# imuncle/TSCM_Calib

Measured on AMD Instinct MI355X. Metric: LM iterations/sec at 4 cams x 10k views (joint intrinsics+extrinsics, fp64), higher is better.
Workload: dtype f64

## Files before the change

### include/tscm/tscm.h

```cpp
#ifndef TSCM_H
#define TSCM_H

#include <stddef.h>

#ifdef __cplusplus
extern "C" {
#endif

#define TSCM_ABI_VERSION 6

enum {
    TSCM_OK = 0,
    TSCM_E_INVALID = -1,
    TSCM_E_NO_DEVICE = -2,
    TSCM_E_HIP = -3,
    TSCM_E_RCCL = -4,
    TSCM_E_UNSUPPORTED = -5,
    TSCM_E_NOMEM = -6,
    TSCM_E_PEER = -7
};

enum { TSCM_CONVERGENCE = 0, TSCM_NO_CONVERGENCE = 1, TSCM_FAILURE = 2 };

#define TSCM_MAX_ITERATIONS 255

typedef struct tscm_problem {
    int n_cameras;
    int n_boards;
    int n_points;
    int n_views;
    const double *board_xy;
    const int *view_camera;
    const int *view_board;
    const int *view_offset;
    const int *view_count;
    const double *obs_u;
    const double *obs_v;
    double *cam_rt;
    double *intr;
    double *board_rt;
    const unsigned char *cam_pose_constant;
    int mono;
    const unsigned char *board_pose_constant;
} tscm_problem;

typedef struct tscm_options {
    size_t struct_size;
    int max_num_iterations;
    double function_tolerance;
    double gradient_tolerance;
    double parameter_tolerance;
    double initial_trust_region_radius;
    double max_trust_region_radius;
    double min_trust_region_radius;
    double min_relative_decrease;
    double min_lm_diagonal;
    double max_lm_diagonal;
    int max_num_consecutive_invalid_steps;
    int jacobi_scaling;
    int check_every;
    int jacobian_fp32;
    int exec_flags;
} tscm_options;

enum {
    TSCM_EXEC_SEPARATE_T_REDUCE = 1,
    TSCM_EXEC_KEEP_SINGLE_RANK_COMM = 2,
    TSCM_EXEC_GRAM_16X16 = 4,
    TSCM_EXEC_SEPARATE_BACKSUB = 8,
    TSCM_EXEC_SEPARATE_CONTROL = 16,
    TSCM_EXEC_DENSE_REDUCED_ORDER = 32,
    TSCM_EXEC_GRAPH_REDUCED_ORDER = 64,
    TSCM_EXEC_SEPARATE_STATS = 128,
    TSCM_EXEC_ALL = 255
};

typedef struct tscm_iteration {
    int iteration;
    int step_is_valid;
    int step_is_successful;
    double cost;
    double cost_change;
    double gradient_max_norm;
    double gradient_norm;
    double step_norm;
    double relative_decrease;
    double trust_region_radius;
} tscm_iteration;

typedef struct tscm_summary {
    int termination_type;
    int num_iterations;
    int num_successful_steps;
    int num_unsuccessful_steps;
    double initial_cost;
    double final_cost;
    int n_residual_blocks;
    int lm_iterations;
    tscm_iteration iterations[TSCM_MAX_ITERATIONS + 1];
    char message[128];
    double seconds_solve;
    double seconds_total;
    double rmse;
} tscm_summary;

typedef struct tscm_solver tscm_solver;
typedef struct tscm_comm tscm_comm;

int tscm_abi_version(void);
const char *tscm_last_error(void);
int tscm_device_count(void);
int tscm_device_synchronize(int device);
int tscm_device_peak_fp64(int device, double *mfma_tflops, double *valu_tflops);
int tscm_device_peak_fp64_ex(int device, double peaks[3]);
int tscm_device_peak_fp32_mfma(int device, double *tflops);

void tscm_default_options(tscm_options *opt, int mono);

int tscm_solver_create(const tscm_problem *problem, int device, tscm_solver **out);
int tscm_solver_set_comm(tscm_solver *s, tscm_comm *comm);
int tscm_solver_debug_withhold_handoff(tscm_solver *s, int on);
int tscm_solver_reruns(const tscm_solver *s);
int tscm_solver_solve(tscm_solver *s, const tscm_options *opt, tscm_summary *summary);
int tscm_solver_upload_params(tscm_solver *s, const double *cam_rt, const double *intr, const double *board_rt);
int tscm_solver_solve_resident(tscm_solver *s, const tscm_options *opt, tscm_summary *summary, int reset);
int tscm_solver_download_params(tscm_solver *s, double *cam_rt, double *intr, double *board_rt);
void tscm_solver_destroy(tscm_solver *s);
// ... 253 lines not shown
```

### tscm_calib_amd/csrc/tscm_exec_plan.h

```cpp
#ifndef TSCM_EXEC_PLAN_H
#define TSCM_EXEC_PLAN_H

#include "tscm_layout.h"

#include <algorithm>
#include <string>

#ifdef __HIPCC__
#define TSCM_PLAN_FN __host__ __device__ inline
#else
#define TSCM_PLAN_FN inline
#endif

namespace tscm {

constexpr int kCamSl = 16;
constexpr int kTSlices = 16;
constexpr int kTEntries = 64;
constexpr int kFusedEntries = 256 / kTSlices;
constexpr int kVPrepThreads = 128;
constexpr int kDense4Cams = 4;

constexpr int kCtlOneGpu = 1;
constexpr int kCtlComm = 2;
constexpr int kCtlInit = 4;
constexpr int kCtlRide = 8;
constexpr int kCtlWithhold = 16;

enum CommKind { kCommNone, kCommOneRank, kCommShared };
inline bool uses_comm(int kind, int exec_flags) { return kind == kCommShared || (kind == kCommOneRank && (exec_flags & TSCM_EXEC_KEEP_SINGLE_RANK_COMM)); }

enum class Gram { G4, F32, G16, G16Pitch58 };
enum class EvalTail {
    ReduceControl,
    StatsThenHead,
    Ride,
    Exchange,
};
enum class Solver { Empty, Dense4, Nd, Big };

struct ExecDevice {
    int schur_resident[4] = {}, schur_resident_ride[4] = {};
    int dense4_resident = 0;
    int nd_resident[2] = {}, nd_tpt[2] = { 1, 1 };
};

struct ExecPlan {
    bool comm = false;
    Gram gram = Gram::G4;
    bool robust = false;
    EvalTail tail = EvalTail::ReduceControl;
    bool ctl_in_schur = false;
    bool stats_ride = false;
    bool t_in_solve = false;
    Solver solver = Solver::Empty;
    int nd = 0, tpt = 1;
    int n_prod = 0, n_bs = 0;
    int bs_threads = 0;
    bool f32() const { return gram == Gram::F32; }
};

inline int reduction_blocks(const Layout &L, int C) { return C * kCamSl + (L.B + 255) / 256; }

inline Gram plan_gram(int exec_flags, int jacobian_fp32, int rp)
{
    if (jacobian_fp32) return Gram::F32;
    if (!(exec_flags & TSCM_EXEC_GRAM_16X16)) return Gram::G4;
    return rp == 58 ? Gram::G16Pitch58 : Gram::G16;
}

constexpr int kG4MaxKS = 14;
struct G4Plan { int passes, per, ks; };
TSCM_PLAN_FN G4Plan g4_plan(int n_points)
{
    G4Plan g;
    g.passes = (n_points + 4 * kG4MaxKS - 1) / (4 * kG4MaxKS);
    if (g.passes < 1) g.passes = 1;
    g.ks = ((n_points + g.passes - 1) / g.passes + 3) / 4;
    if (g.ks < 1) g.ks = 1;
    g.per = 4 * g.ks;
    return g;
}

inline ExecPlan plan_exec(const Layout &L, int C, int n_act, int comm_kind, int exec_flags, int jacobian_fp32, int loss_kind, int rp,
                          const ExecDevice &dev)
{
    ExecPlan p;
    p.comm = uses_comm(comm_kind, exec_flags);
    p.gram = plan_gram(exec_flags, jacobian_fp32, rp);
    p.robust = loss_kind != TSCM_LOSS_NONE;
    const int n_variants = (L.nv_chunks[1] ? 1 : 0) + (L.nv_chunks[2] ? 1 : 0) + (L.nv_chunks[3] ? 1 : 0);
    const bool small = C <= kMaxCamLds;
    p.ctl_in_schur = (p.comm || small) && L.slow_boards.empty() && L.pc_begin.empty() && n_variants == 1 &&
                     !(exec_flags & TSCM_EXEC_SEPARATE_CONTROL);
    const int nv = L.nv_chunks[1] ? 1 : L.nv_chunks[2] ? 2 : 3;
    p.stats_ride = p.ctl_in_schur && !p.comm && small && !(exec_flags & TSCM_EXEC_SEPARATE_STATS) &&
                   std::max(reduction_blocks(L, C), L.nv_chunks[nv]) + 1 <= dev.schur_resident_ride[nv];
    p.tail = p.comm || !small ? EvalTail::Exchange : !p.ctl_in_schur ? EvalTail::ReduceControl : p.stats_ride ? EvalTail::Ride : EvalTail::StatsThenHead;
    p.t_in_solve = !(exec_flags & TSCM_EXEC_SEPARATE_T_REDUCE) && small && !p.comm && L.n_bids > 0 && L.n_bids <= kSmallBids && n_act > 0;
    p.n_prod = p.t_in_solve ? L.n_bids * (256 / kFusedEntries) : 0;
    p.nd = (exec_flags & TSCM_EXEC_DENSE_REDUCED_ORDER) ? 1 : 0;
    const bool graph_order = (exec_flags & TSCM_EXEC_GRAPH_REDUCED_ORDER) || p.nd;
    p.solver = n_act == 0 ? Solver::Empty : C <= kDense4Cams && !graph_order ? Solver::Dense4 : small ? Solver::Nd : Solver::Big;
    if (p.solver != Solver::Nd) p.nd = 0;
    p.tpt = p.solver == Solver::Nd ? dev.nd_tpt[p.nd] : 1;
    if (p.solver == Solver::Dense4 || p.solver == Solver::Nd) {
        const int resident = p.solver == Solver::Dense4 ? dev.dense4_resident : dev.nd_resident[p.nd];
        if (!(exec_flags & TSCM_EXEC_SEPARATE_BACKSUB) && L.bs_threads == 256 && L.n_bs_blocks <= resident - 1 - p.n_prod) p.n_bs = L.n_bs_blocks;
    }
    p.bs_threads = !p.n_bs && L.n_bs_blocks ? L.bs_threads : 0;
    return p;
}

inline int check_exec_options(const tscm_options &o, int loss_kind, std::string &err)
{
    if (o.max_num_iterations < 0 || o.max_num_iterations > TSCM_MAX_ITERATIONS) return layout_fail(err, TSCM_E_INVALID, "max_num_iterations must be in [0, 255]");
    if (o.exec_flags & ~TSCM_EXEC_ALL) return layout_fail(err, TSCM_E_INVALID, "unknown bits in tscm_options.exec_flags (an options struct of an older ABI?)");
    if (loss_kind != TSCM_LOSS_NONE && (o.exec_flags & TSCM_EXEC_GRAM_16X16)) return layout_fail(err, TSCM_E_UNSUPPORTED, "TSCM_EXEC_GRAM_16X16 has no robust-loss kernel");
    return 0;
}

}

#endif
```

### tscm_calib_amd/csrc/tscm_kernels.h

```cpp
#pragma once

#include "tscm_math.h"
#include "tscm_fastmath.h"
#include "tscm_nd_plan.h"
#include "tscm_layout.h"
#include "tscm_exec_plan.h"
#include "tscm_columns.h"
#include "tscm_ctrl.h"

namespace tscm {
#include "tscm_dev.h"
#include "tscm_probe.h"
#include "tscm_prep.h"
#include "tscm_geometry.h"
#include "tscm_eval_gram16.h"
#include "tscm_eval_f32.h"
#include "tscm_eval_gram4.h"
#include "tscm_reduce.h"
#include "tscm_schur.h"
#include "tscm_backsub.h"
#include "tscm_solve_nd.h"
#include "tscm_solve_dense4.h"
#include "tscm_solve_big.h"
#include "tscm_begin_end.h"
#include "tscm_ops.h"

}
```

### tscm_calib_amd/csrc/tscm_schur.h

```cpp
#pragma once

__device__ __forceinline__ bool chol6(const double M[21], double L[21])
{
    bool ok = true;
#pragma unroll
    for (int j = 0; j < 6; ++j) {
        double d = M[j * (j + 1) / 2 + j];
#pragma unroll
        for (int k = 0; k < j; ++k) d -= L[j * (j + 1) / 2 + k] * L[j * (j + 1) / 2 + k];
        if (!(d > 0.0)) { ok = false; d = 1.0; }
        const double inv = fast_rsqrt(d);
        L[j * (j + 1) / 2 + j] = inv;
#pragma unroll
        for (int i = j + 1; i < 6; ++i) {
            double s = M[i * (i + 1) / 2 + j];
#pragma unroll
            for (int k = 0; k < j; ++k) s -= L[i * (i + 1) / 2 + k] * L[j * (j + 1) / 2 + k];
            L[i * (i + 1) / 2 + j] = s * inv;
        }
    }
    return ok;
}

__device__ __forceinline__ bool factor_core(double (&M)[21], const double (&g)[6], const double (&sb)[6], double radius, double dmin, double dmax, double *f,
// ... 58 lines not shown
    if (!factor_core(M, g, sb, radius, dmin, dmax, S.fac + (size_t)kFac * b, P.board_const[b] != 0)) *S.fac_fail = 1;
}

__global__ __launch_bounds__(256) void k_schur_factor(DevProblem P, DevState S)
{
    if (S.ctrl->done) return;
    const int i = blockIdx.x * 256 + threadIdx.x;
    if (i >= P.n_slow) return;
    const int b = P.slow_boards[i];
    factor_board(P, S, S.ctrl->cur, S.ctrl->radius, S.ctrl->opt.min_lm_diagonal, S.ctrl->opt.max_lm_diagonal, b, P.bv_ptr[b], P.bv_ptr[b + 1]);
}



struct FacFwd { double m[15], c[6], z[6]; };
__device__ __forceinline__ void load_fac_fwd(const double *fac, int board, FacFwd &F)
{
    const cptr4 f = (cptr4)(fac + (size_t)kFac * board);
#pragma unroll
    for (int i = 0; i < 15; ++i) F.m[i] = f[kFacM + i];
#pragma unroll
    for (int i = 0; i < 6; ++i) { F.c[i] = f[kFacC + i]; F.z[i] = f[kFacZ + i]; }
}

__device__ __forceinline__ void y_column(const FacFwd &F, const double (&w)[6], bool grad_col, double (&y)[6])
{
    y[0] = F.c[0] * w[0];
    y[1] = F.c[1] * w[1] - F.m[0] * y[0];
    y[2] = F.c[2] * w[2] - F.m[1] * y[0] - F.m[2] * y[1];
    y[3] = F.c[3] * w[3] - F.m[3] * y[0] - F.m[4] * y[1] - F.m[5] * y[2];
    y[4] = F.c[4] * w[4] - F.m[6] * y[0] - F.m[7] * y[1] - F.m[8] * y[2] - F.m[9] * y[3];
    y[5] = F.c[5] * w[5] - F.m[10] * y[0] - F.m[11] * y[1] - F.m[12] * y[2] - F.m[13] * y[3] - F.m[14] * y[4];
#pragma unroll
    for (int i = 0; i < 6; ++i) y[i] = grad_col ? F.z[i] : y[i];
}

__device__ __forceinline__ void y_column_operands(const FacFwd &F, const double (&w)[6], bool grad_col, int kq, double &s0, double &s1)
{
    double y[6];
    y_column(F, w, grad_col, y);
    double y0 = y[0], y1 = y[1], y2 = y[2], y3 = y[3], y4 = y[4], y5 = y[5];
    asm volatile("" : "+v"(y0), "+v"(y1), "+v"(y2), "+v"(y3), "+v"(y4), "+v"(y5));
    const bool lo = (kq & 1) == 0, first = kq < 2;
    const double a01 = lo ? y0 : y1, a23 = lo ? y2 : y3, a45 = lo ? y4 : y5;
    s0 = first ? a01 : a23;
    s1 = first ? a45 : 0.0;
}

struct RawTc {
    const double *r;
    __device__ __forceinline__ double operator[](int i) const { return r[3 * (i / 6 - kWcolTc) + (i % 6 - 3)]; }
};

template <int NV, bool RIDE = false>
__global__ __launch_bounds__(256, RIDE && NV <= 2 ? 2 : 1) void k_schur_gram(DevProblem P, DevState S, int chunk0, int ctl, int first_round, int ctl_epoch, int stats_target, int n_chunks)
{
#ifdef TSCM_WAVE_TIMELINE
    KtlScope ktl_scope(3, ctl && !RIDE ? S.ctrl_snap : static_cast<const CtrlHead *>(S.ctrl));
#endif
    PHASE_STAMP(tsk);
    static_assert(kCtlInit == 1 << 2 && kCtlWithhold == 1 << 4 && (kCtlOneGpu | kCtlComm) == 3, "k_schur_gram's decode of ctl");
    const int ctl_init = (ctl >> 2) & 1, withhold = (ctl >> 4) & 1;
    ctl &= 3;
    const int n_stats = RIDE ? P.C * kCamSl + S.n_st_blocks : 0;
    const int bid = (int)blockIdx.x;
    const bool extra = ctl != 0 && bid == 0;
    const int jblk = ctl ? bid - 1 : bid;
    const int cblk = RIDE ? min(max(jblk, 0), n_chunks - 1) : max(jblk, 0);
    const int4 desc = P.bc_desc[chunk0 + cblk];
    constexpr int NT = NV * (NV + 1) / 2;
    constexpr int NE = 24 + 9 * NV, NJ = (NE + 15) / 16;
    struct __attribute__((aligned(16))) Lds { double facl[kChunkBoards][kFac]; double sumE[kChunkBoards][NE]; double tiles[4][NT][256]; };
    __shared__ Lds lds_blk;
    double (&sumE)[kChunkBoards][NE] = lds_blk.sumE;
    double (&facl)[kChunkBoards][kFac] = lds_blk.facl;
    double (&tiles)[4][NT][256] = lds_blk.tiles;
    const int chunk = chunk0 + cblk;
    const int tid = threadIdx.x;
    const int wave = __builtin_amdgcn_readfirstlane(tid >> 6), lane = tid & 63;
    const int a = lane & 15, kq = lane >> 4;
    const int c0 = desc.x, nbd = desc.y - desc.x, slot0 = desc.z;
    constexpr unsigned BAD = 0xffffe000u;
    double ev[4][NJ];
    double w[4][NV][6];
    const double *Rcp[NV];
    auto request = [&](int cur_) {
        const __amdgpu_buffer_rsrc_t r_w = make_rsrc(S.rec[cur_], sizeof(double) * (size_t)kRec * P.V);
        {
            const int e = tid & 15;
#pragma unroll
            for (int j = 0; j < NJ; ++j) {
                const int idx = e + 16 * j;
                const int pv = idx < 24 ? 0 : (idx - 24) / 9, r9 = idx < 24 ? 0 : (idx - 24) % 9;
                const bool summed = idx < 24;
                const unsigned first = idx < 18 ? 8u * ((unsigned)kRecW * (unsigned)P.V + (unsigned)idx)
                                     : idx < 24 ? 8u * (unsigned)(6 * kFR + idx - 18)
                                     : 8u * (unsigned)(kRecW * pv + 6 * (kWcolTc + r9 / 3) + 3 + r9 % 3);
                const unsigned per_slot = idx < 18 ? 8u * kRecE : 8u * kRecW;
#pragma unroll
                for (int i = 0; i < 4; ++i) {
                    const int bf = 16 * i + (tid >> 4);
                    const unsigned o0 = idx < NE ? first + per_slot * (unsigned)(slot0 + NV * min(bf, nbd - 1)) : BAD;
                    double acc = 0.0;
#pragma unroll
                    for (int p = 0; p < NV; ++p) acc += buf_load_f64(r_w, (p == 0 || summed) ? o0 : BAD, per_slot * (unsigned)p);
                    ev[i][j] = acc;
                }
// ... 155 lines not shown
                    ev[i][j] = acc;
                }
            }
        }
#pragma unroll
        for (int g = 0; g < 4; ++g) {
            const int bg = 16 * wave + 4 * g + kq;
            const unsigned base = (a < 14 && bg < nbd) ? 8u * ((unsigned)kRecW * (unsigned)(slot0 + NV * bg) + 6u * (unsigned)a) : BAD;
#pragma unroll
            for (int p = 0; p < NV; ++p)
#pragma unroll
                for (int k = 0; k < 3; ++k) {
                    const d2 v = buf_load_2f64(r_w, base, 8u * (unsigned)(kRecW * p + 2 * k));
                    w[g][p][2 * k] = v[0]; w[g][p][2 * k + 1] = v[1];
                }
        }
#pragma unroll
        for (int p = 0; p < NV; ++p) Rcp[p] = S.cconst[cur] + kCStride * P.slot_cam[slot0 + p];
    }
    double sb[6];
#pragma unroll
    for (int i = 0; i < 6; ++i) sb[i] = tid < nbd ? S.s_b[6 * (c0 + tid) + i] : 1.0;
    const bool board_is_const = tid < nbd && P.board_const[c0 + tid] != 0;
    {
        const int e = tid & 15, grp = tid >> 4;
#pragma unroll
        for (int i = 0; i < 4; ++i)
#pragma unroll
            for (int j = 0; j < NJ; ++j) if (e + 16 * j < NE) sumE[16 * i + grp][e + 16 * j] = ev[i][j];
    }
    __syncthreads();
    PHASE_STAMP(ts1);
    if (tid < nbd) {
        double M[21], g[6];
#pragma unroll
        for (int i = 0; i < 6; ++i) {
#pragma unroll
            for (int j = 0; j <= i; ++j) {
                if (j < 3) M[i * (i + 1) / 2 + j] = sumE[tid][6 * j + i];
                else {
                    double acc = 0.0;
#pragma unroll
                    for (int p = 0; p < NV; ++p) acc += tb_tb(RawTc{ &sumE[tid][24 + 9 * p] }, Rcp[p], i - 3, j - 3);
                    M[i * (i + 1) / 2 + j] = acc;
                }
            }
            g[i] = sumE[tid][18 + i];
        }
        if (!factor_core(M, g, sb, radius, dmin, dmax, facl[tid], board_is_const)) *S.fac_fail = 1;
    }
    __syncthreads();
    PHASE_STAMP(ts2);
    for (int i = tid; i < nbd * kFac; i += 256) S.fac[(size_t)kFac * c0 + i] = (&facl[0][0])[i];
    d4 acc[NT];
#pragma unroll
    for (int t = 0; t < NT; ++t) acc[t] = d4{ 0.0, 0.0, 0.0, 0.0 };
    const bool grad_col = a == kFR;
#pragma unroll
    for (int g = 0; g < 4; ++g) {
        if (16 * wave + 4 * g >= nbd) break;
        const int bg = 16 * wave + 4 * g + kq;
        const bool valid = bg < nbd;
        const int bl = min(bg, nbd - 1);
        FacFwd F;
#pragma unroll
        for (int i = 0; i < 15; ++i) F.m[i] = facl[bl][kFacM + i];
#pragma unroll
        for (int i = 0; i < 6; ++i) { F.c[i] = facl[bl][kFacC + i]; F.z[i] = valid ? facl[bl][kFacZ + i] : 0.0; }
        double y[NV][6];
#pragma unroll
        for (int p = 0; p < NV; ++p) y_column(F, w[g][p], grad_col, y[p]);
#pragma unroll
        for (int r = 0; r < 6; ++r) {
            int t = 0;
#pragma unroll
            for (int p = 0; p < NV; ++p)
#pragma unroll
                for (int q = p; q < NV; ++q, ++t) acc[t] = __builtin_amdgcn_mfma_f64_16x16x4f64(y[p][r], y[q][r], acc[t], 0, 0, 0);
        }
    }
    PHASE_STAMP(ts3);
#pragma unroll
    for (int t = 0; t < NT; ++t)
#pragma unroll
        for (int r = 0; r < 4; ++r) tiles[wave][t][(kq + 4 * r) * 16 + a] = acc[t][r];
    __syncthreads();
#pragma unroll
    for (int t = 0; t < NT; ++t)
        S.pairpart[(size_t)256 * P.bc_tile[6 * chunk + t] + tid] = (tiles[0][t][tid] + tiles[1][t][tid]) + (tiles[2][t][tid] + tiles[3][t][tid]);
#ifdef TSCM_WAVE_TIMELINE
    if (threadIdx.x == 0 && ktl_scope.on && (int)blockIdx.x < kKtlGroups) {
        long long *o = g_phs + (size_t)kPhStamps * blockIdx.x;
        o[0] = tsk; o[1] = ts0; o[2] = ts1; o[3] = ts2; o[4] = ts3; o[5] = wall_clock64(); o[6] = nbd; o[7] = (bid >= first_round ? 1 : 0) | ((RIDE && t_waited ? t_waited - tsk : 0) << 1) | ((RIDE && t_reduced ? t_reduced - tsk : 0) << 32);
    }
#endif
#ifdef TSCM_PHASE_PROFILE
    if (threadIdx.x == 0 && (cblk == 0 || cblk == 200))
        printf("schur_gram wg %d: boards %d  head %lld  E sums %lld  factor %lld  gram %lld  tiles %lld [10 ns]\n", (int)blockIdx.x, nbd, ts0 - tsk, ts1 - ts0, ts2 - ts1, ts3 - ts2, wall_clock64() - ts3);
#endif
}

__global__ __launch_bounds__(256) void k_pair_gram(DevProblem P, DevState S)
{
    if (S.ctrl->done) return;
    __shared__ double red[4][256];
    const int pc = blockIdx.x;
    const int cur = S.ctrl->cur;
    const int wave = threadIdx.x >> 6, lane = threadIdx.x & 63;
    const int a = lane & 15, kq = lane >> 4;
    d4 acc = { 0.0, 0.0, 0.0, 0.0 };
    for (int p = P.pc_begin[pc] + wave; p < P.pc_end[pc]; p += 4) {
        const double *Wi = rec_w(S.rec[cur], P.pair_i[p]), *Wj = rec_w(S.rec[cur], P.pair_j[p]);
        FacFwd F;
        load_fac_fwd(S.fac, __builtin_amdgcn_readfirstlane(P.pair_board[p]), F);
        double wi[6], wj[6];
#pragma unroll
        for (int k = 0; k < 6; ++k) { wi[k] = a < 14 ? Wi[6 * a + k] : 0.0; wj[k] = a < 14 ? Wj[6 * a + k] : 0.0; }
        double i0, i1, j0, j1;
        y_column_operands(F, wi, a == kFR, kq, i0, i1);
        y_column_operands(F, wj, a == kFR, kq, j0, j1);
        acc = __builtin_amdgcn_mfma_f64_16x16x4f64(i0, j0, acc, 0, 0, 0);
        acc = __builtin_amdgcn_mfma_f64_16x16x4f64(i1, j1, acc, 0, 0, 0);
    }
#pragma unroll
    for (int r = 0; r < 4; ++r) red[wave][(kq + 4 * r) * 16 + a] = acc[r];
    __syncthreads();
    const int t = threadIdx.x;
    S.pairpart[(size_t)256 * P.pc_tile[pc] + t] = (red[0][t] + red[1][t]) + (red[2][t] + red[3][t]);
}

template <int ENTRIES>
__device__ __forceinline__ void t_reduce_block(const DevState &S, int bid, int part, int cb, int ce, double (*red)[ENTRIES])
{
    const int e = threadIdx.x % ENTRIES, slice = threadIdx.x / ENTRIES;
    const int entry = part * ENTRIES + e;
    const int per = (ce - cb + kTSlices - 1) / kTSlices;
    const int b0 = cb + slice * per, b1 = min(ce, b0 + per);
    double a0 = 0.0, a1 = 0.0, a2 = 0.0, a3 = 0.0, a4 = 0.0, a5 = 0.0, a6 = 0.0, a7 = 0.0;
// ... 95 lines not shown
```

### tscm_calib_amd/csrc/tscm_solver.hip

```cpp
#include "tscm/tscm.h"
#include "tscm_host.h"
#include "tscm_kernels.h"
#include "tscm_launch_seq.h"
#include "tscm_mono_batch.h"

#include <hip/hip_runtime.h>
#include <hip/hip_ext.h>
#include <rccl/rccl.h>

#include <algorithm>
#include <chrono>
#include <cstdio>
#include <cstdlib>
#include <cmath>
#include <cstring>
#include <memory>
#include <numeric>
#include <string>
#include <thread>
#include <vector>

using namespace tscm;

static thread_local std::string g_err;
// ... 254 lines not shown
    if (fixed) for (int m = 0; m < C; ++m) if (fixed[m] & ~TSCM_FIX_ALL) return fail(TSCM_E_INVALID, "unknown bits in a fixed-intrinsics mask (bits 0-8 only)");
    return 0;
}

extern "C" int tscm_solver_set_fixed_intrinsics(tscm_solver *s, const unsigned short *fixed)
{
    if (!s) return fail(TSCM_E_INVALID, "solver is NULL");
    if (int rc = check_fixed(fixed, s->C)) return rc;
    std::vector<unsigned short> f(s->C, 0);
    if (fixed) f.assign(fixed, fixed + s->C);
    if (f == s->fixed) return 0;
    ColumnPlan c;
    std::string err;
    if (int rc = plan_columns(s->L, s->C, f.data(), c, err)) return fail(rc, err);
    if (int rc = apply_columns(s, c)) return rc;
    s->fixed = f;
    return 0;
}

extern "C" int tscm_solver_create_sharded(const tscm_problem *p, int device, int rank, int world, tscm_solver **out)
{
    if (!out) return fail(TSCM_E_INVALID, "out is NULL");
    *out = nullptr;
    if (int rc = validate(p)) return rc;
    if (world < 1 || rank < 0 || rank >= world) return fail(TSCM_E_INVALID, "rank / world out of range");
    if (int rc = select_device(device, "the TSCM solver")) return rc;

    SolverPtr sp(new tscm_solver);
    tscm_solver *s = sp.get();
    s->device = device;
    s->rank = rank; s->world = world;
    s->C = p->n_cameras; s->n_points = p->n_points; s->mono = p->mono != 0;
    s->n_pad = 16 * s->C;
    s->h_cam_rt = p->cam_rt; s->h_intr = p->intr; s->h_board_rt = p->board_rt;
    HIP_TRY(hipStreamCreateWithFlags(&s->stream, hipStreamNonBlocking));
    s->own_stream = s->stream;
    const int C = s->C;

    const int half_rows = 8 * ((std::min(64, p->n_points) + 7) / 8);
    const int rp = half_rows + 2;
    const size_t lds_eval_bytes = sizeof(double) * (std::max<size_t>((size_t)16 * rp, 512) + kCst + 2 * (size_t)p->n_points);
    if (4 * lds_eval_bytes > 64 * 1024) HIP_TRY(hipFuncSetAttribute(reinterpret_cast<const void *>(k_eval_gram<0>), hipFuncAttributeMaxDynamicSharedMemorySize, (int)(4 * lds_eval_bytes)));
    const G4Plan g4 = g4_plan(p->n_points);
    const EvalKernel eval4 = g4_kernel(g4.ks, g4.passes > 1, false), eval4r = g4_kernel(g4.ks, g4.passes > 1, true);
    const size_t lds_eval4 = 4 * sizeof(double) * (size_t)eval_gram4_lds_doubles(p->n_points, g4.ks);
    if (lds_eval4 > 160 * 1024) return fail(TSCM_E_UNSUPPORTED, "board with too many corners for the Gram kernel's LDS (more than about 2,000)");
    if (lds_eval4 > 64 * 1024)
        for (EvalKernel k : { eval4, eval4r }) HIP_TRY(hipFuncSetAttribute(reinterpret_cast<const void *>(k), hipFuncAttributeMaxDynamicSharedMemorySize, (int)lds_eval4));
    int wgs_per_cu = 0;
    HIP_TRY(hipOccupancyMaxActiveBlocksPerMultiprocessor(&wgs_per_cu, reinterpret_cast<const void *>(eval4), 256, lds_eval4));
    const int waves_per_cu = 4 * std::max(1, std::min(4, wgs_per_cu));
    hipDeviceProp_t prop;
    HIP_TRY(hipGetDeviceProperties(&prop, device));
    const void *schur[4][2] = { {}, { reinterpret_cast<const void *>(k_schur_gram<1>), reinterpret_cast<const void *>(k_schur_gram<1, true>) },
                                { reinterpret_cast<const void *>(k_schur_gram<2>), reinterpret_cast<const void *>(k_schur_gram<2, true>) },
                                { reinterpret_cast<const void *>(k_schur_gram<3>), reinterpret_cast<const void *>(k_schur_gram<3, true>) } };
    for (int nv = 1; nv <= 3; ++nv) {
        HIP_TRY(hipOccupancyMaxActiveBlocksPerMultiprocessor(&s->dev.schur_resident[nv], schur[nv][0], 256, 0));
        HIP_TRY(hipOccupancyMaxActiveBlocksPerMultiprocessor(&s->dev.schur_resident_ride[nv], schur[nv][1], 256, 0));
        s->dev.schur_resident[nv] *= prop.multiProcessorCount; s->dev.schur_resident_ride[nv] *= prop.multiProcessorCount;
    }
    s->n_cu = std::max(1, prop.multiProcessorCount);

    const Layout &L = s->L;
    {
        LayoutDevice dev;
        dev.n_cu = prop.multiProcessorCount; dev.waves_per_cu = waves_per_cu;
        std::string err;
        if (int rc = plan_layout(p, rank, world, dev, s->L, err)) return fail(rc, err);
    }
    s->B = L.B; s->V = L.V; s->N = L.N;
    const int B = L.B, V = L.V, N = L.N;
    s->lds_bs = sizeof(double) * (size_t)(L.bs_threads == 256 ? BsGeom<256>::kLds : BsGeom<128>::kLds);
    for (const void *k : { reinterpret_cast<const void *>(k_backsub_prep<128>), reinterpret_cast<const void *>(k_backsub_prep<256>) })
        HIP_TRY(hipFuncSetAttribute(k, hipFuncAttributeMaxDynamicSharedMemorySize, (int)s->lds_bs));

    std::vector<double> u((size_t)N), w((size_t)N);
    for (int i = 0; i < V; ++i) {
        const int v = L.dev2orig[i];
        std::memcpy(u.data() + L.view_obs[i], p->obs_u + p->view_offset[v], sizeof(double) * L.view_count[i]);
        std::memcpy(w.data() + L.view_obs[i], p->obs_v + p->view_offset[v], sizeof(double) * L.view_count[i]);
    }
    const std::vector<double> bxy(p->board_xy, p->board_xy + 2 * (size_t)p->n_points);
    auto int4s = [](const std::vector<Int4> &h) {
        std::vector<int4> d(h.size());
        for (size_t i = 0; i < h.size(); ++i) d[i] = make_int4(h[i].x, h[i].y, h[i].z, h[i].w);
        return d;
    };
    const std::vector<int4> chunk_desc = int4s(L.chunk_desc), bc_desc = int4s(L.bc_desc);
    const std::vector<short> bid_lut(L.bid_of.begin(), L.bid_of.end());
    DevProblem &P = s->P;
    DevState &S = s->S;
    P.C = C; P.B = B; P.n_points = p->n_points; P.V = V; P.N = N; P.n_pad = s->n_pad;
    P.rank = rank; P.world = world;
    P.rp = rp; P.half = half_rows; P.lds_wave = (int)(lds_eval_bytes / sizeof(double)); P.g4_per = g4.per;
    P.n_chunks = (int)L.chunk_vb.size(); P.n_pchunks = (int)L.pc_begin.size(); P.n_bids = L.n_bids;
    P.n_bchunks = (int)L.bc_desc.size(); P.n_tiles = L.n_tiles; P.n_slow = (int)L.slow_boards.size();
    std::copy(std::begin(L.cam_wg), std::end(L.cam_wg), P.cam_wg);
    std::copy(std::begin(L.bid_part_small), std::end(L.bid_part_small), P.bid_part_small);
    P.pair_mask = L.pair_mask;
    hipError_t he = hipSuccess;
    auto up = [&](auto **dst, const auto &h) { if (he == hipSuccess) he = s->mem.upload(dst, h); };
    auto al = [&](auto **dst, size_t n) { if (he == hipSuccess) he = s->mem.alloc(dst, n); };
    up(&P.board_xy, bxy);
    up(&P.view_cam, L.view_cam); up(&P.view_board, L.view_board); up(&P.view_obs, L.view_obs); up(&P.view_count, L.view_count);
    up(&P.obs_u, u); up(&P.obs_v, w);
    up(&P.chunk_vb, L.chunk_vb); up(&P.chunk_ve, L.chunk_ve); up(&P.chunk_cam, L.chunk_cam); up(&P.chunk_desc, chunk_desc);
    up(&P.cam_chunk_ptr, L.cam_chunk_ptr);
    up(&P.bv_ptr, L.bv_ptr); up(&P.view_slot, L.view_slot); up(&P.slot_cam, L.slot_cam); up(&P.slot_view, L.slot_view); up(&P.slot_board, L.slot_board);
    up(&P.slow_boards, L.slow_boards);
    up(&P.pair_i, L.pair_i); up(&P.pair_j, L.pair_j); up(&P.pc_begin, L.pc_begin); up(&P.pc_end, L.pc_end); up(&P.pc_tile, L.pc_tile);
    up(&P.bid_part_ptr, L.bid_part_ptr); up(&P.pair_board, L.pair_board); up(&P.bc_tile, L.bc_tile); up(&P.bc_desc, bc_desc);
    up(&P.bid_lut, bid_lut); up(&P.board_const, L.board_const);
// ... 255 lines not shown
            hipLaunchKernelGGL(k_ipc_allreduce, dim3(1), dim3(1024), 0, stream, buf + off, m, peers, x->rank, x->world, x->max_doubles, ++x->count, x->d_fault);
        }
        return 0;
    }
    NCCL_TRY(ncclAllReduce(buf, buf, n, ncclDouble, ncclSum, c->comm, stream));
    return 0;
}
static int comm_check(tscm_comm *c)
{
    if (!c || !c->ipc) return 0;
    int f = 0;
    HIP_TRY(hipMemcpy(&f, c->ipc->d_fault, sizeof(int), hipMemcpyDeviceToHost));
    if (f) { c->ipc->dead = true; return fail(TSCM_E_PEER, "IPC exchange: a peer rank did not arrive within the bound (failed or gone); the communicator is unusable from here on"); }
    return 0;
}

struct LmSeq {
    SeqState st;
    LaunchList todo;
    int at = 0;
};
struct LmRun {
    std::vector<tscm_solver *> m;
    std::vector<LmSeq> seq;
};

static int exchange(LmRun &run, bool t_buffer)
{
    tscm_solver *s0 = run.m[0];
    if (!s0->comm) return 0;
    const size_t n = t_buffer ? 256 * (size_t)s0->P.n_bids : 256 * (size_t)s0->P.C + kScal + s0->P.world;
    if (n == 0) return 0;
    hipEvent_t e1 = nullptr;
    if (s0->comm->group) {
        tscm_local_group *g = s0->comm->group;
        if (int rc = timed_begin(s0, t_buffer ? 1 : 2, g->stream, &e1)) return rc;
        hipLaunchKernelGGL(k_xchg_sum, dim3((unsigned)((n + 255) / 256)), dim3(256), 0, g->stream, g->d_ptrs + (t_buffer ? 0 : g->world), g->world, n);
        if (e1) HIP_TRY(hipEventRecord(e1, g->stream));
        return 0;
    }
    double *buf = t_buffer ? s0->S.T : s0->S.H_stage;
    if (int rc = timed_begin(s0, t_buffer ? 1 : 2, s0->stream, &e1)) return rc;
    if (int rc = comm_allreduce(s0->comm, buf, n, s0->stream)) return rc;
    if (e1) HIP_TRY(hipEventRecord(e1, s0->stream));
    return 0;
}

static int enqueue(tscm_solver *s, const Launch &l)
{
    const DevProblem &P = s->P;
    const DevState &S = s->S;
    hipStream_t st = s->stream;
    const dim3 grid(l.grid);
    auto schur = [&](auto kernel) { hipLaunchKernelGGL(kernel, grid, dim3(256), 0, st, P, S, l.chunk0, l.ctl, l.first_round, l.ce, l.target, l.n_chunks); };
    auto nd = [&](auto kernel) {
        const int v = l.nd;
        hipLaunchKernelGGL(kernel, grid, dim3(kNdThreads), std::max(s->lds_nd[v], l.n_bs ? s->lds_bs : (size_t)0), st, P, S, s->d_nd_map[v], s->d_nd_tab[v], s->d_nd_bs[v],
                           s->plan[v].dims(), l.epoch, l.withhold, l.n_prod, l.n_bs, l.f32);
    };
    const size_t lds_dense4 = std::max(s->lds_dense4, l.n_bs ? s->lds_bs : (size_t)0);
    switch (l.k) {
    case Kern::BeginViewPrep: {
        const bool init = l.start == Start::Init, bak = l.start == Start::Backup;
        hipLaunchKernelGGL(k_begin_view_prep, grid, dim3(kVPrepThreads), 0, st, P, S, s->head,
                           init ? s->d_init_cam : bak ? s->d_start_cam : nullptr, init ? s->d_init_intr : bak ? s->d_start_intr : nullptr,
                           init ? s->d_init_board : bak ? s->d_start_board : nullptr,
                           bak ? nullptr : s->d_start_cam, bak ? nullptr : s->d_start_intr, bak ? nullptr : s->d_start_board, l.f32);
        break;
    }
    case Kern::Eval: return launch_eval(s, l.cand);
    case Kern::ReduceControl: hipLaunchKernelGGL(k_reduce_control, grid, dim3(256), 0, st, P, S, l.cand, l.init, l.have_backsub); break;
    case Kern::ReduceStats: hipLaunchKernelGGL(k_reduce_stats, grid, dim3(256), 0, st, P, S, l.cand, l.init); break;
    case Kern::FinalizeEval: hipLaunchKernelGGL(k_finalize_eval, grid, dim3(256), 0, st, P, S, l.have_backsub); break;
    case Kern::Control: hipLaunchKernelGGL(k_control, grid, dim3(256), 0, st, P, S, l.init); break;
    case Kern::SchurFactor: hipLaunchKernelGGL(k_schur_factor, grid, dim3(256), 0, st, P, S); break;
    case Kern::Schur1: schur(k_schur_gram<1>); break;
    case Kern::Schur2: schur(k_schur_gram<2>); break;
    case Kern::Schur3: schur(k_schur_gram<3>); break;
    case Kern::SchurRide1: schur(k_schur_gram<1, true>); break;
    case Kern::SchurRide2: schur(k_schur_gram<2, true>); break;
    case Kern::SchurRide3: schur(k_schur_gram<3, true>); break;
    case Kern::PairGram: hipLaunchKernelGGL(k_pair_gram, grid, dim3(256), 0, st, P, S); break;
    case Kern::TReduce: hipLaunchKernelGGL(k_T_reduce, grid, dim3(kTEntries * kTSlices), 0, st, P, S); break;
    case Kern::SolveDense4: hipLaunchKernelGGL((k_solve_reduced<4, 16, 64>), grid, dim3(256), lds_dense4, st, P, S, l.epoch, l.withhold, l.n_prod, l.n_bs, l.f32); break;
    case Kern::SolveDense4Ride: hipLaunchKernelGGL((k_solve_reduced<4, 16, 64, true>), grid, dim3(256), lds_dense4, st, P, S, l.epoch, l.withhold, l.n_prod, l.n_bs, l.f32); break;
    case Kern::SolveNd1: nd(k_solve_nd<1, false>); break;
    case Kern::SolveNd2: nd(k_solve_nd<2, false>); break;
    case Kern::SolveNd1Ride: nd(k_solve_nd<1, true>); break;
    case Kern::SolveNd2Ride: nd(k_solve_nd<2, true>); break;
    case Kern::SolveBig: hipLaunchKernelGGL(k_solve_reduced_big, grid, dim3(kBigNT), s->lds_solve, st, P, S); break;
    case Kern::SolveEmpty: hipLaunchKernelGGL(k_solve_reduced_big, grid, dim3(kBigNT), solve_big_lds_bytes(0, s->n_pad), st, P, S); break;
    case Kern::Backsub128: hipLaunchKernelGGL(k_backsub_prep<128>, grid, dim3(128), s->lds_bs, st, P, S, l.f32); break;
    case Kern::Backsub256: hipLaunchKernelGGL(k_backsub_prep<256>, grid, dim3(256), s->lds_bs, st, P, S, l.f32); break;
    case Kern::FinishSolve: hipLaunchKernelGGL(k_finish_solve, grid, dim3(256), 0, st, P, S, l.init, l.have_backsub, s->C, s->B, s->d_h_ctrl); break;
    case Kern::EndSolve: hipLaunchKernelGGL(k_end_solve, grid, dim3(256), 0, st, S, s->C, s->B); break;
    case Kern::CopyCtrl: {
        static_assert(sizeof(Ctrl) == sizeof(CtrlHead) + sizeof(IterLog) * kMaxLog, "the log follows the head without padding");
        const size_t bytes = sizeof(CtrlHead) + sizeof(IterLog) * (size_t)std::min(s->head.opt.max_num_iterations + 1, kMaxLog);
        HIP_TRY(hipMemcpyAsync(s->h_ctrl, S.ctrl, bytes, hipMemcpyDeviceToHost, st));
        break;
    }
    case Kern::ExchangeT: case Kern::ExchangeH: break;
    }
    return 0;
}

static int walk(LmRun &run)
{
    for (LmSeq &q : run.seq) q.at = 0;
    for (bool left = true; left;) {
        left = false;
        const Launch *mark = nullptr;
        for (size_t r = 0; r < run.m.size(); ++r) {
            LmSeq &q = run.seq[r];
            for (const int from = q.at; q.at < q.todo.n; ++q.at) {
                const Launch &l = q.todo.at[q.at];
                if (is_exchange(l.k) || (l.k == Kern::Eval && q.at > from)) break;
                if (int rc = enqueue(run.m[r], l)) return rc;
            }
            if (q.at < q.todo.n && is_exchange(q.todo.at[q.at].k)) mark = &q.todo.at[q.at++];
            left = left || q.at < q.todo.n;
        }
        if (mark) if (int rc = exchange(run, mark->k == Kern::ExchangeT)) return rc;
    }
    return 0;
}

static const char *reason_message(int r)
{
    switch (r) {
    case kMaxIter: return "Maximum number of iterations reached.";
    case kGradTol: return "Gradient tolerance reached.";
    case kMinRadius: return "Minimum trust region radius reached.";
    case kParamTol: return "Parameter tolerance reached.";
// ... 928 lines not shown
```

### tscm_calib_amd/lib.py

```python
from __future__ import annotations

import ctypes as C
import os
import subprocess

import numpy as np

_HERE = os.path.dirname(os.path.abspath(__file__))
CSRC = os.path.join(_HERE, "csrc")
LIB_PATH = os.path.join(CSRC, "libtscm_hip.so")
UNIQUE_ID_BYTES = 128
IPC_HANDLE_BYTES = 80
MAX_ITERATIONS = 255
EXEC_SEPARATE_T_REDUCE = 1
EXEC_KEEP_SINGLE_RANK_COMM = 2
EXEC_GRAM_16X16 = 4
EXEC_SEPARATE_BACKSUB = 8
EXEC_SEPARATE_CONTROL = 16
EXEC_DENSE_REDUCED_ORDER = 32
EXEC_GRAPH_REDUCED_ORDER = 64
EXEC_SEPARATE_STATS = 128
LOSS_NONE, LOSS_HUBER, LOSS_SOFT_L1, LOSS_CAUCHY = 0, 1, 2, 3
LOSS_KINDS = {None: LOSS_NONE, "none": LOSS_NONE, "huber": LOSS_HUBER, "soft_l1": LOSS_SOFT_L1, "cauchy": LOSS_CAUCHY}
PROJ_PERSPECTIVE, PROJ_LONGLAT, PROJ_CYLINDRICAL, PROJ_STEREOGRAPHIC, PROJ_EQUIRECT = 0, 1, 2, 3, 4
PROJ_KINDS = {"perspective": PROJ_PERSPECTIVE, "longlat": PROJ_LONGLAT, "cylindrical": PROJ_CYLINDRICAL,
              "stereographic": PROJ_STEREOGRAPHIC, "equirect": PROJ_EQUIRECT}
PANO_SEAM, PANO_FEATHER, PANO_MULTIBAND = 0, 1, 2
PANO_MODES = {"seam": PANO_SEAM, "feather": PANO_FEATHER, "multiband": PANO_MULTIBAND}
INTRINSIC_NAMES = ("fx", "fy", "cx", "cy", "xi", "lambda", "alpha", "b", "c")
FIX = {name: 1 << k for k, name in enumerate(INTRINSIC_NAMES)}
FIX_INTRINSICS, FIX_ALL = 127, 511
MODEL_DS = FIX["lambda"]
MODEL_UCM = FIX["xi"] | FIX["lambda"]

E_NAMES = {0: "TSCM_OK", -1: "TSCM_E_INVALID", -2: "TSCM_E_NO_DEVICE", -3: "TSCM_E_HIP",
           -4: "TSCM_E_RCCL", -5: "TSCM_E_UNSUPPORTED", -6: "TSCM_E_NOMEM", -7: "TSCM_E_PEER"}
TERMINATION = {0: "CONVERGENCE", 1: "NO_CONVERGENCE", 2: "FAILURE"}


class TscmError(RuntimeError):
    def __init__(self, code: int, message: str):
        super().__init__(f"{E_NAMES.get(code, code)}: {message}")
        self.code = code


class CProblem(C.Structure):
    _fields_ = [
        ("n_cameras", C.c_int), ("n_boards", C.c_int), ("n_points", C.c_int), ("n_views", C.c_int),
        ("board_xy", C.c_void_p), ("view_camera", C.c_void_p), ("view_board", C.c_void_p),
        ("view_offset", C.c_void_p), ("view_count", C.c_void_p), ("obs_u", C.c_void_p), ("obs_v", C.c_void_p),
        ("cam_rt", C.c_void_p), ("intr", C.c_void_p), ("board_rt", C.c_void_p),
        ("cam_pose_constant", C.c_void_p), ("mono", C.c_int), ("board_pose_constant", C.c_void_p),
    ]


class COptions(C.Structure):
    _fields_ = [
        ("struct_size", C.c_size_t), ("max_num_iterations", C.c_int), ("function_tolerance", C.c_double), ("gradient_tolerance", C.c_double),
        ("parameter_tolerance", C.c_double), ("initial_trust_region_radius", C.c_double),
        ("max_trust_region_radius", C.c_double), ("min_trust_region_radius", C.c_double),
        ("min_relative_decrease", C.c_double), ("min_lm_diagonal", C.c_double), ("max_lm_diagonal", C.c_double),
        ("max_num_consecutive_invalid_steps", C.c_int), ("jacobi_scaling", C.c_int), ("check_every", C.c_int),
        ("jacobian_fp32", C.c_int), ("exec_flags", C.c_int),
    ]


class CIteration(C.Structure):
    _fields_ = [
        ("iteration", C.c_int), ("step_is_valid", C.c_int), ("step_is_successful", C.c_int),
        ("cost", C.c_double), ("cost_change", C.c_double), ("gradient_max_norm", C.c_double),
        ("gradient_norm", C.c_double), ("step_norm", C.c_double), ("relative_decrease", C.c_double),
        ("trust_region_radius", C.c_double),
    ]

# ... 299 lines not shown
```

Measured before the change: 8741.

## Compute Schur Gram tiles with 4x4x4 f64 MFMA and DPP rotations by default

The default Schur Gram accumulation now uses 4x4x4 f64 MFMA instructions, feeding rotated B operands through DPP lane shuffles. On diagonal tiles it skips the redundant symmetric rotations and mirrors the results into the LDS tile. The old 16x16x4 MFMA path stays available behind a new TSCM_EXEC_SCHUR_16X16 flag, and occupancy is taken as the minimum over both variants. The aim is to avoid wasted MFMA work on symmetric blocks and to use a smaller accumulator footprint, at the cost of DPP shuffles and scattered LDS stores.

```diff
diff --git a/include/tscm/tscm.h b/include/tscm/tscm.h
--- a/include/tscm/tscm.h
+++ b/include/tscm/tscm.h
@@ -72,7 +72,8 @@
     TSCM_EXEC_DENSE_REDUCED_ORDER = 32,
     TSCM_EXEC_GRAPH_REDUCED_ORDER = 64,
     TSCM_EXEC_SEPARATE_STATS = 128,
-    TSCM_EXEC_ALL = 255
+    TSCM_EXEC_SCHUR_16X16 = 512,
+    TSCM_EXEC_ALL = 255 | 512
 };
 
 typedef struct tscm_iteration {
diff --git a/tscm_calib_amd/csrc/tscm_exec_plan.h b/tscm_calib_amd/csrc/tscm_exec_plan.h
--- a/tscm_calib_amd/csrc/tscm_exec_plan.h
+++ b/tscm_calib_amd/csrc/tscm_exec_plan.h
@@ -49,6 +49,7 @@
     bool comm = false;
     Gram gram = Gram::G4;
     bool robust = false;
+    bool schur16 = false;
     EvalTail tail = EvalTail::ReduceControl;
     bool ctl_in_schur = false;
     bool stats_ride = false;
@@ -89,6 +90,7 @@
     p.comm = uses_comm(comm_kind, exec_flags);
     p.gram = plan_gram(exec_flags, jacobian_fp32, rp);
     p.robust = loss_kind != TSCM_LOSS_NONE;
+    p.schur16 = (exec_flags & TSCM_EXEC_SCHUR_16X16) != 0;
     const int n_variants = (L.nv_chunks[1] ? 1 : 0) + (L.nv_chunks[2] ? 1 : 0) + (L.nv_chunks[3] ? 1 : 0);
     const bool small = C <= kMaxCamLds;
     p.ctl_in_schur = (p.comm || small) && L.slow_boards.empty() && L.pc_begin.empty() && n_variants == 1 &&
diff --git a/tscm_calib_amd/csrc/tscm_kernels.h b/tscm_calib_amd/csrc/tscm_kernels.h
--- a/tscm_calib_amd/csrc/tscm_kernels.h
+++ b/tscm_calib_amd/csrc/tscm_kernels.h
@@ -5,6 +5,7 @@
 #include "tscm_nd_plan.h"
 #include "tscm_layout.h"
 #include "tscm_exec_plan.h"
+#include "tscm_schur_sched.h"
 #include "tscm_columns.h"
 #include "tscm_ctrl.h"
 
diff --git a/tscm_calib_amd/csrc/tscm_schur.h b/tscm_calib_amd/csrc/tscm_schur.h
--- a/tscm_calib_amd/csrc/tscm_schur.h
+++ b/tscm_calib_amd/csrc/tscm_schur.h
@@ -134,7 +134,28 @@
     __device__ __forceinline__ double operator[](int i) const { return r[3 * (i / 6 - kWcolTc) + (i % 6 - 3)]; }
 };
 
-template <int NV, bool RIDE = false>
+template <int NV, int K = 0>
+__device__ __forceinline__ void schur_gram4_row(const double (&ya)[NV], const double (&yb)[NV][4], double (&acc)[sg_instr_count(NV)])
+{
+    if constexpr (K < sg_instr_count(NV)) {
+        constexpr SgInstr in = sg_instr(NV, K);
+        acc[K] = __builtin_amdgcn_mfma_f64_4x4x4f64(ya[in.p], yb[in.q][in.rot], acc[K], 0, 0, 0);
+        schur_gram4_row<NV, K + 1>(ya, yb, acc);
+    }
+}
+template <int NV, int K = 0>
+__device__ __forceinline__ void schur_gram4_store(const double (&acc)[sg_instr_count(NV)], double (*tile)[256], int lane)
+{
+    if constexpr (K < sg_instr_count(NV)) {
+        constexpr SgInstr in = sg_instr(NV, K);
+        const int row = sg_row(lane), col = sg_col(lane, in.rot), use = sg_use(in.p == in.q, in.rot, sg_block(lane));
+        if (use != kSgUnused) tile[in.tile][16 * row + col] = acc[K];
+        if (use == kSgMirrored) tile[in.tile][16 * col + row] = acc[K];
+        schur_gram4_store<NV, K + 1>(acc, tile, lane);
+    }
+}
+
+template <int NV, bool RIDE = false, bool G16 = false>
 __global__ __launch_bounds__(256, RIDE && NV <= 2 ? 2 : 1) void k_schur_gram(DevProblem P, DevState S, int chunk0, int ctl, int first_round, int ctl_epoch, int stats_target, int n_chunks)
 {
 #ifdef TSCM_WAVE_TIMELINE
@@ -396,9 +417,16 @@
     __syncthreads();
     PHASE_STAMP(ts2);
     for (int i = tid; i < nbd * kFac; i += 256) S.fac[(size_t)kFac * c0 + i] = (&facl[0][0])[i];
-    d4 acc[NT];
-#pragma unroll
-    for (int t = 0; t < NT; ++t) acc[t] = d4{ 0.0, 0.0, 0.0, 0.0 };
+    constexpr int NI = sg_instr_count(NV);
+    d4 acc[G16 ? NT : 1];
+    double acc4[G16 ? 1 : NI];
+    if constexpr (G16) {
+#pragma unroll
+        for (int t = 0; t < NT; ++t) acc[t] = d4{ 0.0, 0.0, 0.0, 0.0 };
+    } else {
+#pragma unroll
+        for (int k = 0; k < NI; ++k) acc4[k] = 0.0;
+    }
     const bool grad_col = a == kFR;
 #pragma unroll
     for (int g = 0; g < 4; ++g) {
@@ -416,18 +444,34 @@
         for (int p = 0; p < NV; ++p) y_column(F, w[g][p], grad_col, y[p]);
 #pragma unroll
         for (int r = 0; r < 6; ++r) {
-            int t = 0;
-#pragma unroll
-            for (int p = 0; p < NV; ++p)
-#pragma unroll
-                for (int q = p; q < NV; ++q, ++t) acc[t] = __builtin_amdgcn_mfma_f64_16x16x4f64(y[p][r], y[q][r], acc[t], 0, 0, 0);
+            if constexpr (G16) {
+                int t = 0;
+#pragma unroll
+                for (int p = 0; p < NV; ++p)
+#pragma unroll
+                    for (int q = p; q < NV; ++q, ++t) acc[t] = __builtin_amdgcn_mfma_f64_16x16x4f64(y[p][r], y[q][r], acc[t], 0, 0, 0);
+            } else {
+                double yb[NV][4];
+#pragma unroll
+                for (int q = 0; q < NV; ++q) {
+                    yb[q][0] = y[q][r]; yb[q][1] = dpp_f64<0x12C>(y[q][r]); yb[q][2] = dpp_f64<0x128>(y[q][r]); yb[q][3] = dpp_f64<0x124>(y[q][r]);
+                }
+                double ya[NV];
+#pragma unroll
+                for (int p = 0; p < NV; ++p) ya[p] = y[p][r];
+                schur_gram4_row<NV>(ya, yb, acc4);
+            }
         }
     }
     PHASE_STAMP(ts3);
-#pragma unroll
-    for (int t = 0; t < NT; ++t)
-#pragma unroll
-        for (int r = 0; r < 4; ++r) tiles[wave][t][(kq + 4 * r) * 16 + a] = acc[t][r];
+    if constexpr (G16) {
+#pragma unroll
+        for (int t = 0; t < NT; ++t)
+#pragma unroll
+            for (int r = 0; r < 4; ++r) tiles[wave][t][(kq + 4 * r) * 16 + a] = acc[t][r];
+    } else {
+        schur_gram4_store<NV>(acc4, tiles[wave], lane);
+    }
     __syncthreads();
 #pragma unroll
     for (int t = 0; t < NT; ++t)
diff --git a/tscm_calib_amd/csrc/tscm_schur_sched.h b/tscm_calib_amd/csrc/tscm_schur_sched.h
--- /dev/null
+++ b/tscm_calib_amd/csrc/tscm_schur_sched.h
@@ -0,0 +1,42 @@
+#ifndef TSCM_SCHUR_SCHED_H
+#define TSCM_SCHUR_SCHED_H
+
+#ifdef __HIPCC__
+#define TSCM_SCHED_FN __host__ __device__ constexpr
+#else
+#define TSCM_SCHED_FN constexpr
+#endif
+
+namespace tscm {
+
+constexpr int kSgMaxViews = 3;
+struct SgInstr { int p, q, rot, tile; };
+enum SgUse { kSgUnused = 0, kSgDirect = 1, kSgMirrored = 2 };
+
+TSCM_SCHED_FN int sg_tiles(int nv) { return nv * (nv + 1) / 2; }
+TSCM_SCHED_FN int sg_tile(int nv, int p, int q) { return p * nv - p * (p - 1) / 2 + (q - p); }
+TSCM_SCHED_FN int sg_instr_count(int nv) { return 3 * nv + 4 * (nv * (nv - 1) / 2); }
+TSCM_SCHED_FN SgInstr sg_instr(int nv, int k)
+{
+    for (int p = 0; p < nv; ++p)
+        for (int q = p; q < nv; ++q) {
+            const int n = p == q ? 3 : 4;
+            if (k < n) return SgInstr{ p, q, k, sg_tile(nv, p, q) };
+            k -= n;
+        }
+    return SgInstr{ -1, -1, -1, -1 };
+}
+TSCM_SCHED_FN int sg_cgroup(int b, int rot) { return (b + rot) & 3; }
+TSCM_SCHED_FN int sg_use(bool diagonal, int rot, int b)
+{
+    if (!diagonal || rot == 0) return kSgDirect;
+    if (rot == 1) return kSgMirrored;
+    return b < 2 ? kSgMirrored : kSgUnused;
+}
+TSCM_SCHED_FN int sg_block(int lane) { return (lane >> 2) & 3; }
+TSCM_SCHED_FN int sg_row(int lane) { return 4 * sg_block(lane) + (lane >> 4); }
+TSCM_SCHED_FN int sg_col(int lane, int rot) { return 4 * sg_cgroup(sg_block(lane), rot) + (lane & 3); }
+TSCM_SCHED_FN int sg_b_source(int lane, int rot) { return (lane & ~15) | ((lane + 4 * rot) & 15); }
+
+}
+#endif
diff --git a/tscm_calib_amd/csrc/tscm_solver.hip b/tscm_calib_amd/csrc/tscm_solver.hip
--- a/tscm_calib_amd/csrc/tscm_solver.hip
+++ b/tscm_calib_amd/csrc/tscm_solver.hip
@@ -330,13 +330,16 @@
     const int waves_per_cu = 4 * std::max(1, std::min(4, wgs_per_cu));
     hipDeviceProp_t prop;
     HIP_TRY(hipGetDeviceProperties(&prop, device));
-    const void *schur[4][2] = { {}, { reinterpret_cast<const void *>(k_schur_gram<1>), reinterpret_cast<const void *>(k_schur_gram<1, true>) },
-                                { reinterpret_cast<const void *>(k_schur_gram<2>), reinterpret_cast<const void *>(k_schur_gram<2, true>) },
-                                { reinterpret_cast<const void *>(k_schur_gram<3>), reinterpret_cast<const void *>(k_schur_gram<3, true>) } };
+#define TSCM_SCHUR_PAIR(NV, RIDE) { reinterpret_cast<const void *>(k_schur_gram<NV, RIDE>), reinterpret_cast<const void *>(k_schur_gram<NV, RIDE, true>) }
+    const void *schur[4][2][2] = { {}, { TSCM_SCHUR_PAIR(1, false), TSCM_SCHUR_PAIR(1, true) }, { TSCM_SCHUR_PAIR(2, false), TSCM_SCHUR_PAIR(2, true) },
+                                   { TSCM_SCHUR_PAIR(3, false), TSCM_SCHUR_PAIR(3, true) } };
+#undef TSCM_SCHUR_PAIR
     for (int nv = 1; nv <= 3; ++nv) {
-        HIP_TRY(hipOccupancyMaxActiveBlocksPerMultiprocessor(&s->dev.schur_resident[nv], schur[nv][0], 256, 0));
-        HIP_TRY(hipOccupancyMaxActiveBlocksPerMultiprocessor(&s->dev.schur_resident_ride[nv], schur[nv][1], 256, 0));
-        s->dev.schur_resident[nv] *= prop.multiProcessorCount; s->dev.schur_resident_ride[nv] *= prop.multiProcessorCount;
+        int res[2][2];
+        for (int ride = 0; ride < 2; ++ride)
+            for (int g16 = 0; g16 < 2; ++g16) HIP_TRY(hipOccupancyMaxActiveBlocksPerMultiprocessor(&res[ride][g16], schur[nv][ride][g16], 256, 0));
+        s->dev.schur_resident[nv] = std::min(res[0][0], res[0][1]) * prop.multiProcessorCount;
+        s->dev.schur_resident_ride[nv] = std::min(res[1][0], res[1][1]) * prop.multiProcessorCount;
     }
     s->n_cu = std::max(1, prop.multiProcessorCount);
 
@@ -698,7 +701,9 @@
     const DevState &S = s->S;
     hipStream_t st = s->stream;
     const dim3 grid(l.grid);
-    auto schur = [&](auto kernel) { hipLaunchKernelGGL(kernel, grid, dim3(256), 0, st, P, S, l.chunk0, l.ctl, l.first_round, l.ce, l.target, l.n_chunks); };
+    auto schur = [&](auto kernel, auto kernel16) {
+        hipLaunchKernelGGL(s->xp.schur16 ? kernel16 : kernel, grid, dim3(256), 0, st, P, S, l.chunk0, l.ctl, l.first_round, l.ce, l.target, l.n_chunks);
+    };
     auto nd = [&](auto kernel) {
         const int v = l.nd;
         hipLaunchKernelGGL(kernel, grid, dim3(kNdThreads), std::max(s->lds_nd[v], l.n_bs ? s->lds_bs : (size_t)0), st, P, S, s->d_nd_map[v], s->d_nd_tab[v], s->d_nd_bs[v],
@@ -720,12 +725,12 @@
     case Kern::FinalizeEval: hipLaunchKernelGGL(k_finalize_eval, grid, dim3(256), 0, st, P, S, l.have_backsub); break;
     case Kern::Control: hipLaunchKernelGGL(k_control, grid, dim3(256), 0, st, P, S, l.init); break;
     case Kern::SchurFactor: hipLaunchKernelGGL(k_schur_factor, grid, dim3(256), 0, st, P, S); break;
-    case Kern::Schur1: schur(k_schur_gram<1>); break;
-    case Kern::Schur2: schur(k_schur_gram<2>); break;
-    case Kern::Schur3: schur(k_schur_gram<3>); break;
-    case Kern::SchurRide1: schur(k_schur_gram<1, true>); break;
-    case Kern::SchurRide2: schur(k_schur_gram<2, true>); break;
-    case Kern::SchurRide3: schur(k_schur_gram<3, true>); break;
+    case Kern::Schur1: schur(k_schur_gram<1>, k_schur_gram<1, false, true>); break;
+    case Kern::Schur2: schur(k_schur_gram<2>, k_schur_gram<2, false, true>); break;
+    case Kern::Schur3: schur(k_schur_gram<3>, k_schur_gram<3, false, true>); break;
+    case Kern::SchurRide1: schur(k_schur_gram<1, true>, k_schur_gram<1, true, true>); break;
+    case Kern::SchurRide2: schur(k_schur_gram<2, true>, k_schur_gram<2, true, true>); break;
+    case Kern::SchurRide3: schur(k_schur_gram<3, true>, k_schur_gram<3, true, true>); break;
     case Kern::PairGram: hipLaunchKernelGGL(k_pair_gram, grid, dim3(256), 0, st, P, S); break;
     case Kern::TReduce: hipLaunchKernelGGL(k_T_reduce, grid, dim3(kTEntries * kTSlices), 0, st, P, S); break;
     case Kern::SolveDense4: hipLaunchKernelGGL((k_solve_reduced<4, 16, 64>), grid, dim3(256), lds_dense4, st, P, S, l.epoch, l.withhold, l.n_prod, l.n_bs, l.f32); break;
diff --git a/tscm_calib_amd/lib.py b/tscm_calib_amd/lib.py
--- a/tscm_calib_amd/lib.py
+++ b/tscm_calib_amd/lib.py
@@ -20,6 +20,7 @@
 EXEC_DENSE_REDUCED_ORDER = 32
 EXEC_GRAPH_REDUCED_ORDER = 64
 EXEC_SEPARATE_STATS = 128
+EXEC_SCHUR_16X16 = 512
 LOSS_NONE, LOSS_HUBER, LOSS_SOFT_L1, LOSS_CAUCHY = 0, 1, 2, 3
 LOSS_KINDS = {None: LOSS_NONE, "none": LOSS_NONE, "huber": LOSS_HUBER, "soft_l1": LOSS_SOFT_L1, "cauchy": LOSS_CAUCHY}
 PROJ_PERSPECTIVE, PROJ_LONGLAT, PROJ_CYLINDRICAL, PROJ_STEREOGRAPHIC, PROJ_EQUIRECT = 0, 1, 2, 3, 4
```

After: 8802 (median of 6 runs). No clear change (+0.7%).
